# locuslab/icnn

Hardware: AMD Instinct MI355X
Metric: inner-solves/sec (batch x iters), n=159 K=10 (higher is better)
Workload: dtype f32 PICNN / f64 dual solve

## Files before the change

### icnn_amd/csrc/be_common.h

```cpp
#pragma once
#ifndef ICNN_BE_PROF
#define ICNN_BE_PROF 0
#endif
#define ICNN_BE_PROF_ON(p) (ICNN_BE_PROF && (p))
#include <hip/hip_runtime.h>
#include <stdint.h>

namespace icnn_be {

typedef double d4 __attribute__((ext_vector_type(4)));
typedef float f4 __attribute__((ext_vector_type(4)));

constexpr int WAVE = 64;

__device__ __forceinline__ int thread_id() {
    int t = threadIdx.x;
    asm volatile("" : "+v"(t));
    return t;
}

__device__ __forceinline__ int lane_id() { return (int)__builtin_amdgcn_mbcnt_hi(~0u, __builtin_amdgcn_mbcnt_lo(~0u, 0u)); }

__device__ __forceinline__ double wave_sum(double v) {
#pragma unroll
    for (int o = 32; o > 0; o >>= 1) v += __shfl_xor(v, o);
    return v;
}
__device__ __forceinline__ double wave_max(double v) {
#pragma unroll
    for (int o = 32; o > 0; o >>= 1) v = fmax(v, __shfl_xor(v, o));
    return v;
}
__device__ __forceinline__ float wave_sum_f(float v) {
#pragma unroll
    for (int o = 32; o > 0; o >>= 1) v += __shfl_xor(v, o);
    return v;
}

template <int CTRL> __device__ __forceinline__ float dpp_move(float x) {
    return __builtin_bit_cast(float, __builtin_amdgcn_update_dpp(0, __builtin_bit_cast(int, x), CTRL, 0xF, 0xF, true));
}
template <int CTRL> __device__ __forceinline__ double dpp_move(double x) {
    const int lo = __builtin_amdgcn_update_dpp(0, __double2loint(x), CTRL, 0xF, 0xF, true);
    const int hi = __builtin_amdgcn_update_dpp(0, __double2hiint(x), CTRL, 0xF, 0xF, true);
    return __hiloint2double(hi, lo);
}
template <typename T> __device__ __forceinline__ T sum8_numpy_order(T r) {
    r = r + dpp_move<0xB1>(r);
    r = r + dpp_move<0x4E>(r);
    r = r + dpp_move<0x141>(r);
    return r;
}

constexpr int PW_MAX_LEAVES = 64;
constexpr int PW_MAX_PROG = 2 * PW_MAX_LEAVES;
struct PairwisePlan {
    int n_leaves;
    int n_prog;
    int depth;
    short leaf_start[PW_MAX_LEAVES];
    short leaf_len[PW_MAX_LEAVES];
    signed char prog[PW_MAX_PROG];
};

inline void pw_build_rec(PairwisePlan &p, int start, int n, int level) {
    if (n <= 128) {
        p.leaf_start[p.n_leaves] = (short)start;
        p.leaf_len[p.n_leaves] = (short)n;
        p.prog[p.n_prog++] = (signed char)p.n_leaves;
        if (p.n_leaves == 0) p.depth = level;
        else if (p.depth != level) p.depth = -1;
        p.n_leaves++;
        return;
    }
    int n2 = n / 2;
    n2 -= n2 % 8;
    pw_build_rec(p, start, n2, level + 1);
    pw_build_rec(p, start + n2, n - n2, level + 1);
    p.prog[p.n_prog++] = -1;
}
inline bool pw_build(PairwisePlan &p, int n) {
    p.n_leaves = 0;
    p.n_prog = 0;
    p.depth = -1;
    if (n > 128 * PW_MAX_LEAVES / 2) return false;
    pw_build_rec(p, 0, n, 0);
    if (p.depth > 4 || p.n_leaves != (1 << (p.depth < 0 ? 0 : p.depth))) p.depth = -1;
    return true;
}

template <int NW>
__device__ __forceinline__ void sample_sync() {
    if (NW == 1) {
        __builtin_amdgcn_fence(__ATOMIC_SEQ_CST, "wavefront");
        __builtin_amdgcn_wave_barrier();
    } else {
        __syncthreads();
    }
}

template <int NW, typename T, typename Plan, typename Elem>
__device__ void np_pairwise_rows(const Plan &plan, int rows, Elem elem, T *leafbuf, T *out, int tid) {
    const int lane = tid;
    const int grp = tid >> 3, c = tid & 7;
    const int ngrp = (64 * NW) >> 3;
    const int tasks = rows * plan.n_leaves;
    for (int base = 0; base < tasks; base += ngrp) {
        const int task = base + grp;
        const bool live = task < tasks;
        const int r = live ? task / plan.n_leaves : 0;
        const int lf = live ? task - r * plan.n_leaves : 0;
        const int st = plan.leaf_start[lf], len = plan.leaf_len[lf];
        T res = (T)0;
        if (len < 8) {
            for (int i = 0; i < len; ++i) res = res + elem(r, st + i);
        } else {
            const int body = len - (len % 8);
            T acc = elem(r, st + c);
            int i = 8;
            for (; i + 32 <= body; i += 32) {
                const T e0 = elem(r, st + i + c), e1 = elem(r, st + i + 8 + c), e2 = elem(r, st + i + 16 + c),
                        e3 = elem(r, st + i + 24 + c);
                acc = acc + e0;
                acc = acc + e1;
                acc = acc + e2;
                acc = acc + e3;
            }
            for (; i < body; i += 8) acc = acc + elem(r, st + i + c);
            res = sum8_numpy_order(acc);
            for (i = body; i < len; ++i) res = res + elem(r, st + i);
        }
        if (live && c == 0) leafbuf[task] = res;
    }
    sample_sync<NW>();
    if (plan.depth >= 0) {
        const int depth = plan.depth, L = plan.n_leaves, total = rows * L;
        for (int base = 0; base < total; base += 64 * NW) {
            const int t = base + tid;
            T v = t < total ? leafbuf[t] : (T)0;
            if (depth >= 1) v = v + dpp_move<0xB1>(v);
            if (depth >= 2) v = v + dpp_move<0x4E>(v);
            if (depth >= 3) v = v + dpp_move<0x141>(v);
            if (depth >= 4) v = v + dpp_move<0x140>(v);
            if (t < total && (t & (L - 1)) == 0) out[t >> depth] = v;
        }
        sample_sync<NW>();
        return;
    }
    if (lane < rows) {
        T s0 = 0, s1 = 0, s2 = 0, s3 = 0, s4 = 0, s5 = 0, s6 = 0, s7 = 0;
        int sp = 0;
        for (int i = 0; i < plan.n_prog; ++i) {
            const int tok = plan.prog[i];
            if (tok >= 0) {
                const T v = leafbuf[lane * plan.n_leaves + tok];
                switch (sp) {
                case 0: s0 = v; break; case 1: s1 = v; break; case 2: s2 = v; break; case 3: s3 = v; break;
                case 4: s4 = v; break; case 5: s5 = v; break; case 6: s6 = v; break; default: s7 = v; break;
                }
                ++sp;
            } else {
                switch (sp) {
                case 2: s0 = s0 + s1; break; case 3: s1 = s1 + s2; break; case 4: s2 = s2 + s3; break;
                case 5: s3 = s3 + s4; break; case 6: s4 = s4 + s5; break; case 7: s5 = s5 + s6; break;
                default: s6 = s6 + s7; break;
                }
                --sp;
            }
        }
        out[lane] = s0;
    }
    sample_sync<NW>();
}

}
```

### icnn_amd/csrc/be_dual_dev.h

```cpp
#pragma once
#include <hip/hip_runtime.h>
#include <math.h>
#include <type_traits>

#include "be_common.h"
#include "be_kernels.h"
#include "icnn_be.h"

namespace icnn_be {

namespace {

constexpr double BOUND_EPS = 1e-12;
constexpr double ARMIJO_ALPHA = 1e-5;
constexpr double GRAD_TOL = 1e-10;
constexpr double TINY = 1e-10;
constexpr double CYCLE_TOL = 1e-13;
constexpr double NOISE_TOL = 1e-10;
constexpr int NOISE_T0 = 12;
constexpr int ACCEL_T0 = 24;
constexpr int ACCEL_GAP = 6;
constexpr double ACCEL_NEG_RESID = 1e-10;
constexpr double ACCEL_D2MAX = 1e-3;
constexpr double ACCEL_RMAX = 0.98;
// ... 697 lines not shown
        M1[s] = Hm[(i1 < k ? i1 : 0) * HP + jc];
    }
#pragma unroll
    for (int s = 0; s < NS; ++s) { pin(M0[s]); pin(M1[s]); }
#pragma unroll
    for (int s = 0; s < NS; ++s) {
        const int j = 4 * s + q;
        M0[s] = (i0 < k && j < k) ? M0[s] - (j == i0 ? mu : 0.0) : (j == i0 ? 1.0 : 0.0);
        M1[s] = (i1 < k && j < k) ? M1[s] - (j == i1 ? mu : 0.0) : (j == i1 ? 1.0 : 0.0);
    }
    double dp0 = 1.0, dp1 = 1.0;
    static_for<0, KS>([&](auto P) {
        constexpr int p = decltype(P)::value, qp = p & 3, sp = p >> 2, rp = p & 15;
        constexpr bool upper = p >= 16;
        const double d = row_bcast<rp>(upper ? M1[sp] : M0[sp]);
        const double inv = rcp_nr(d);
        double nf0 = 0.0, nf1;
        if constexpr (!upper) {
            dp0 = (q == qp && i0 == p) ? d : dp0;
            nf0 = quarter_bcast<qp>(i0 > p ? -(M0[sp] * inv) : 0.0);
            nf1 = quarter_bcast<qp>(-(M1[sp] * inv));
        } else {
            dp1 = (q == qp && i1 == p) ? d : dp1;
            nf1 = quarter_bcast<qp>(i1 > p ? -(M1[sp] * inv) : 0.0);
        }
        static_for<sp, NS>([&](auto S) {
            constexpr int s = decltype(S)::value;
            const double pr = row_bcast<rp>(upper ? M1[s] : M0[s]);
            if constexpr (!upper) M0[s] = __builtin_fma(nf0, pr, M0[s]);
            M1[s] = __builtin_fma(nf1, pr, M1[s]);
        });
        __builtin_amdgcn_sched_barrier(0);
    });
    const bool own = (r & 3) == q;
    auto fold = [](unsigned long long m) -> unsigned { return (unsigned)((m | (m >> 16) | (m >> 32) | (m >> 48)) & 0xffffull); };
    unsigned nonpos = fold(__ballot(own && !(dp0 > 0.0))) | (fold(__ballot(own && !(dp1 > 0.0))) << 16);
    unsigned zero = fold(__ballot(own && dp0 == 0.0)) | (fold(__ballot(own && dp1 == 0.0)) << 16);
    const unsigned live = k >= 32 ? 0xffffffffu : ((1u << k) - 1u);
    nonpos &= live; zero &= live;
    if (zero) {
        const int p0 = __builtin_ctz(zero);
        return __popc(nonpos & ((2u << p0) - 1u)) + (k - p0 - 1);
    }
    return __popc(nonpos);
}

template <int KT>
__device__ __forceinline__ int inertia_not_above(const double *Hm, int HP, int k, double mu) {
    if (k <= 4) return inertia_not_above_dpp<4>(Hm, HP, k, mu);
    if (k <= 6) return inertia_not_above_dpp<6>(Hm, HP, k, mu);
    if (k <= 8) return inertia_not_above_dpp<8>(Hm, HP, k, mu);
    if (k <= 10) return inertia_not_above_dpp<10>(Hm, HP, k, mu);
    if (k <= 12) return inertia_not_above_dpp<12>(Hm, HP, k, mu);
    if (KT == 16 || k <= 16) return inertia_not_above_dpp<16>(Hm, HP, k, mu);
    if constexpr (KT > 16) {
        if (k <= 20) return inertia_not_above_2d<20>(Hm, HP, k, mu);
        if (k <= 24) return inertia_not_above_2d<24>(Hm, HP, k, mu);
        return inertia_not_above_2d<32>(Hm, HP, k, mu);
    }
    return 0;
}
__device__ __forceinline__ StepResult newton_step_tri(const double *P, int k, int piv, unsigned long long fmask, bool is_free,
                                                      double g0) {
    if (k <= 4) return newton_step_dpp<4, true>(P, 0, k, piv, fmask, is_free, g0);
    if (k <= 6) return newton_step_dpp<6, true>(P, 0, k, piv, fmask, is_free, g0);
    return newton_step_dpp<8, true>(P, 0, k, piv, fmask, is_free, g0);
}
template <int KT>
__device__ __forceinline__ StepResult newton_step(const double *Hm, int HP, int k, int piv, unsigned long long fmask,
                                                  bool is_free, double g0) {
    if (k <= 4) return newton_step_dpp<4>(Hm, HP, k, piv, fmask, is_free, g0);
    if (k <= 6) return newton_step_dpp<6>(Hm, HP, k, piv, fmask, is_free, g0);
    if (k <= 8) return newton_step_dpp<8>(Hm, HP, k, piv, fmask, is_free, g0);
    if (k <= 10) return newton_step_dpp<10>(Hm, HP, k, piv, fmask, is_free, g0);
    if (k <= 12) return newton_step_dpp<12>(Hm, HP, k, piv, fmask, is_free, g0);
    if (KT == 16 || k <= 16) return newton_step_dpp<16>(Hm, HP, k, piv, fmask, is_free, g0);
    if constexpr (KT > 16) {
        if (k <= 20) return newton_step_2d<20>(Hm, HP, k, piv, fmask, is_free, g0);
        if (k <= 24) return newton_step_2d<24>(Hm, HP, k, piv, fmask, is_free, g0);
        return newton_step_2d<32>(Hm, HP, k, piv, fmask, is_free, g0);
    }
    return StepResult{0.0, 0};
}

template <typename Op>
__device__ __forceinline__ double row16_reduce(double v, Op op) {
    v = op(v, dpp_move<0xB1>(v));
    v = op(v, dpp_move<0x4E>(v));
    v = op(v, dpp_move<0x141>(v));
    v = op(v, dpp_move<0x140>(v));
    return uni(v);
}

template <int KT, typename Op>
__device__ __forceinline__ double rows_reduce(double v, int k, Op op) {
    v = op(v, dpp_move<0xB1>(v));
    v = op(v, dpp_move<0x4E>(v));
    v = op(v, dpp_move<0x141>(v));
    v = op(v, dpp_move<0x140>(v));
    if (KT == 16 || k <= 16) return uni(v);
    return op(bcast(v, 0), bcast(v, 16));
}

template <typename CutT, int NC, typename F>
__device__ __forceinline__ void columns_nc(const CutT *As, int ldA, int k, int zrow, int n_pad, int nt, int tid,
                                           double lam, F &&fin) {
    double acc[NC];
    int jc[NC];
#pragma unroll
    for (int c = 0; c < NC; ++c) {
        const int j = tid + c * nt;
        jc[c] = j < n_pad ? j : n_pad - 1;
        acc[c] = 0.0;
    }
    int i0 = 0;
    for (; i0 + 4 <= k; i0 += 4) {
        CutT av[4][NC];
        double li[4];
#pragma unroll
        for (int d = 0; d < 4; ++d) {
            li[d] = bcast(lam, i0 + d);
#pragma unroll
            for (int c = 0; c < NC; ++c) av[d][c] = As[(i0 + d) * ldA + jc[c]];
        }
#pragma unroll
        for (int d = 0; d < 4; ++d)
#pragma unroll
            for (int c = 0; c < NC; ++c) acc[c] += li[d] * (double)av[d][c];
    }
    for (; i0 < k; ++i0) {
        const double li = bcast(lam, i0);
#pragma unroll
        for (int c = 0; c < NC; ++c) acc[c] += li * (double)As[i0 * ldA + jc[c]];
    }
#pragma unroll
    for (int c = 0; c < NC; ++c) fin(tid + c * nt, tid + c * nt < n_pad, acc[c]);
}
template <typename CutT, typename F>
__device__ __forceinline__ void for_columns(const CutT *As, int ldA, int k, int zrow, int n_pad, int nt, int tid,
                                            double lam, F &&fin) {
    const int per_thread = (n_pad + nt - 1) / nt;
    if (per_thread == 3) columns_nc<CutT, 3>(As, ldA, k, zrow, n_pad, nt, tid, lam, fin);
    else if (per_thread <= 2) columns_nc<CutT, 2>(As, ldA, k, zrow, n_pad, nt, tid, lam, fin);
    else if (per_thread == 4) columns_nc<CutT, 4>(As, ldA, k, zrow, n_pad, nt, tid, lam, fin);
    else
        for (int j0 = 0; j0 < n_pad; j0 += 4 * nt)
            columns_nc<CutT, 4>(As + j0, ldA, k, zrow, n_pad - j0, nt, tid, lam,
                                [&](int j, bool valid, double aj) { fin(j0 + j, valid, aj); });
}

#include "be_dual_valu_dev.h"
#include "be_ipm_dev.h"

template <typename CutT, int KT, int NW, bool RL, bool IPM = false, bool GLB = false, int LR = 0, bool SLICED = true, typename ArgsT>
__device__ __forceinline__ void dual_step_body(const ArgsT &a, int u, int tid, unsigned char *smem, int round,
                                               int rows_cap, const CutT *crow_shared) {
    constexpr int NT = 64 * NW;
    const auto &st = a.st;
    const int lane = tid & 63, wave = tid >> 6;
    const bool w0 = wave == 0;
    auto wg_any = [&](bool p) -> bool { return NW == 1 ? (bool)__any(p) : (bool)__syncthreads_or(p); };
    auto combine = [&](double *Hm_, const double *Hp_, int HP_, int k_, int ncols) {
        if (NW == 1) return;
        sample_sync<NW>();
        for (int e = tid; e < k_ * ncols; e += NT) {
            const int r = e / ncols, c = e - r * ncols;
            double acc = 0.0;
            for (int w = 0; w < NW; ++w) acc += Hp_[(w * rows_cap + r) * HP_ + c];
            Hm_[r * HP_ + c] = acc;
        }
    };
    long long tick = ICNN_BE_PROF_ON(a.prof) ? (long long)__builtin_readcyclecounter() : 0;
    const int T = st.slots;
    const int TI = st.iters > 0 ? st.iters : T;
    const int finished_u = st.finished[u], t_raw = st.t_next[u], phase_u = st.phase[u], cnt_raw = st.count[u];
    const int slot_pre = tid < T ? st.active[(size_t)u * T + tid] : 0;
    const int slot_lane = NW == 1 ? slot_pre : (lane < T ? st.active[(size_t)u * T + lane] : 0);
    if (finished_u) return;
    const int t = __builtin_amdgcn_readfirstlane(t_raw);
    if (t >= TI) return;
    const bool resume = SLICED && __builtin_amdgcn_readfirstlane(phase_u) != 0;

    const int n = st.n, n_pad = a.n_pad, ldA = a.ldA;
    const int HP = (rows_cap + 1) | 1;
    static_assert(!IPM || !RL, "interior point is a variant of its own");
    const Carve cv = carve(KT, rows_cap, ldA, n_pad, (int)sizeof(CutT), a.plan.n_leaves, RL, NW, crow_shared == nullptr, IPM, GLB);
    const int cchunk = NW == 1 ? n_pad : (((n_pad / 16 + NW - 1) / NW) * 16);
    const int cbeg = wave * cchunk < n_pad ? wave * cchunk : n_pad;
    const int cend = cbeg + cchunk < n_pad ? cbeg + cchunk : n_pad;
    CutT *As = GLB ? static_cast<CutT *>(st.scratch) + (size_t)u * (st.slots + 2) * ldA : reinterpret_cast<CutT *>(smem + cv.As);
    static_assert(LR == 0 || GLB, "split staging belongs to the device-memory rounds");
    CutT *AsL = reinterpret_cast<CutT *>(smem + ((cv.total + 15) & ~15));
    const bool mirror = LR > 0 && rows_cap <= HV_KMAX;
    double *zs = reinterpret_cast<double *>(smem + cv.zs);
    double *ws = reinterpret_cast<double *>(smem + cv.ws);
    double *sp = reinterpret_cast<double *>(smem + cv.sp);
    double *Hm = reinterpret_cast<double *>(smem + cv.Hm);
    double *Hp = reinterpret_cast<double *>(smem + cv.Hp) + (NW == 1 ? 0 : wave * rows_cap * HP);
    double *Hp0 = reinterpret_cast<double *>(smem + cv.Hp);
    double *leaf = Hm;
    double *psum = Hm + KT * a.plan.n_leaves;
    int *slots = reinterpret_cast<int *>(smem + cv.ints);

    const CutT *g_row = static_cast<const CutT *>(a.g) + (size_t)u * n;
    const double f_u = (sizeof(CutT) == 4 && (st.flags & ICNN_BE_FLAG_F64_ENERGY))
                           ? static_cast<const double *>(a.f)[u] : (double)static_cast<const CutT *>(a.f)[u];
    double *y_row = st.y + (size_t)u * n;
    CutT *G_u = static_cast<CutT *>(st.G) + (size_t)u * T * n;
    double *ys_u = st.ys + (size_t)u * T * n;
    double *h_u = st.h + (size_t)u * T;

    const int cnt = __builtin_amdgcn_readfirstlane(cnt_raw);
    const int k = cnt + 1;
    if (k > rows_cap) {
        if (tid == 0) {
            st.status[u] |= ICNN_BE_ST_OVERFLOW;
            st.finished[u] = 1;
            st.skip_fg[u] = 1;
        }
        return;
    }
    auto lap = [&](int phase) {
        if (ICNN_BE_PROF_ON(a.prof)) {
            const long long now = (long long)__builtin_readcyclecounter();
            if (tid == 0)
                atomicAdd(reinterpret_cast<unsigned long long *>(a.prof) + (size_t)u * DUAL_PROF_PHASES + phase,
                          (unsigned long long)(now - tick));
            tick = now;
        }
    };
    lap(12);
    int slot_new = t;
    if (TI > T) {
        unsigned used = 0;
        for (int i = 0; i < cnt; ++i) used |= 1u << __builtin_amdgcn_readlane(slot_lane, i);
        slot_new = __builtin_ctz(~used);
    }
    if (tid < cnt) slots[tid] = slot_pre;
    if (tid == cnt) slots[tid] = slot_new;
    const double h_old = lane < cnt ? h_u[slot_lane] : 0.0;
    if (NW > 1) sample_sync<NW>();

    const int per_row = (n_pad + NT - 1) / NT;
    constexpr int MAXC = 4;
    auto stage_older = [&]() {
        if constexpr (NW == 1 && !GLB && LR == 0 && sizeof(CutT) == 4) {
            if (per_row <= MAXC) {
                for (int r = 0; r < cnt; ++r) {
                    const CutT *src = G_u + (size_t)uni(slots[r]) * n;
#pragma unroll
                    for (int c = 0; c < MAXC; ++c) {
                        const int j = tid + c * 64;
                        if (c < per_row && j < n)
                            __builtin_amdgcn_global_load_lds((const __attribute__((address_space(1))) void *)(src + j),
                                                             (__attribute__((address_space(3))) void *)(As + r * ldA + c * 64), 4, 0, 0);
                    }
                }
                for (int j = n + tid; j < n_pad; j += 64)
                    for (int r = 0; r < cnt; ++r) As[r * ldA + j] = (CutT)0;
                __builtin_amdgcn_s_waitcnt(0x0f70);
                return;
            }
        }
        if (per_row <= MAXC) {
            constexpr int RB = 4;
            for (int r0 = 0; r0 < cnt; r0 += RB) {
                CutT v[RB][MAXC];
#pragma unroll
                for (int rr = 0; rr < RB; ++rr) {
                    const bool rok = r0 + rr < cnt;
                    const CutT *src = G_u + (size_t)(rok ? slots[r0 + rr] : 0) * n;
#pragma unroll
                    for (int c = 0; c < MAXC; ++c) {
                        const int j = tid + c * NT;
                        v[rr][c] = rok && c < per_row && j < n ? src[j] : (CutT)0;
                    }
                }
#pragma unroll
                for (int rr = 0; rr < RB; ++rr)
#pragma unroll
                    for (int c = 0; c < MAXC; ++c) {
                        const int j = tid + c * NT;
                        if (r0 + rr < cnt && c < per_row && j < n_pad) {
                            As[(r0 + rr) * ldA + j] = v[rr][c];
                            if (LR > 0 && mirror && r0 + rr < LR) AsL[(r0 + rr) * ldA + j] = v[rr][c];
                        }
                    }
            }
            return;
        }
        const int chunks = cnt * per_row;
#pragma unroll 4
        for (int c = 0; c < chunks; ++c) {
            const int r = c / per_row, j = (c - r * per_row) * NT + tid;
            if (j < n_pad) {
                const CutT v = j < n ? G_u[(size_t)slots[r] * n + j] : (CutT)0;
                As[r * ldA + j] = v;
                if (LR > 0 && mirror && r < LR) AsL[r * ldA + j] = v;
            }
        }
    };
    double h_new;
    if (!resume) {
        bool bad = !isfinite(f_u);
        if (per_row <= MAXC) {
            CutT gr[MAXC];
            double yr[MAXC];
#pragma unroll
            for (int c = 0; c < MAXC; ++c) {
                const int j = tid + c * NT;
                gr[c] = j < n ? g_row[j] : (CutT)0;
                yr[c] = j < n ? y_row[j] : 0.0;
            }
            stage_older();
#pragma unroll
            for (int c = 0; c < MAXC; ++c) {
                const int j = tid + c * NT;
                if (j < n) {
                    G_u[(size_t)slot_new * n + j] = gr[c];
                    ys_u[(size_t)slot_new * n + j] = yr[c];
                    bad |= !isfinite((double)gr[c]);
                }
                if (j < n_pad) {
                    As[cnt * ldA + j] = gr[c];
                    if (LR > 0 && mirror && cnt < LR) AsL[cnt * ldA + j] = gr[c];
                    sp[j] = (double)gr[c] * yr[c];
                }
            }
        } else {
            for (int j = tid; j < n_pad; j += NT) {
                double prod = 0.0;
                if (j < n) {
                    const CutT gj = g_row[j];
                    const double yj = y_row[j];
                    G_u[(size_t)slot_new * n + j] = gj;
                    ys_u[(size_t)slot_new * n + j] = yj;
                    prod = (double)gj * yj;
                    bad |= !isfinite((double)gj);
                    As[cnt * ldA + j] = gj;
                    if (LR > 0 && mirror && cnt < LR) AsL[cnt * ldA + j] = gj;
                } else {
                    As[cnt * ldA + j] = (CutT)0;
                    if (LR > 0 && mirror && cnt < LR) AsL[cnt * ldA + j] = (CutT)0;
                }
                sp[j] = prod;
            }
            stage_older();
        }
        sample_sync<NW>();
        lap(13);
        np_pairwise_rows<NW, double>(a.plan, 1, [&](int, int j) { return sp[j]; }, leaf, psum, tid);
        h_new = f_u - psum[0];
        if (tid == 0) {
            h_u[slot_new] = h_new;
            if (st.fvals) st.fvals[(size_t)u * T + slot_new] = f_u;
        }
        if (wg_any(bad)) {
            if (tid == 0) { st.status[u] |= ICNN_BE_ST_NONFINITE; st.finished[u] = 1; st.skip_fg[u] = 1; }
            return;
        }
    } else {
        for (int j = tid; j < n_pad; j += NT) {
            const CutT v = j < n ? G_u[(size_t)slot_new * n + j] : (CutT)0;
            As[cnt * ldA + j] = v;
            if (LR > 0 && mirror && cnt < LR) AsL[cnt * ldA + j] = v;
        }
        h_new = h_u[slot_new];
        stage_older();
    }
    lap(0);
    const CutT *crow = crow_shared ? crow_shared : As + rows_cap * ldA;
    if (!crow_shared)
        for (int j = tid; j < ldA; j += NT) { As[rows_cap * ldA + j] = (CutT)0; As[(rows_cap + 1) * ldA + j] = (CutT)1; }
    const double h_i = lane < cnt ? h_old : h_new;
    const bool hv_on = !(st.flags & ICNN_BE_FLAG_MFMA_CONTRACTION);
    const int hv_p = hv_pitch(k);
    const bool valu = hv_on && (NW > 1 || (n_pad <= 192 && sizeof(CutT) == 4 && k <= HV_K1MAX)) && !RL && !IPM && k >= 2 &&
                      k <= HV_KMAX && (LR == 0 || mirror) && n_pad <= 256 * NW && NW * hv_p <= n_pad;
    double *hv_part = zs;
    const HvEntry hv_first = hv_entry<true>(lane, k, HP);
    sample_sync<NW>();

    lap(1);
    if (!RL && !resume) {
        bool deficient = false;
        const double cfac = (double)(k > n ? k : n) * Cut<CutT>::eps;
        if (k == 1) {
            bool nz = false;
            for (int j = tid; j < n; j += NT) nz |= As[j] != (CutT)0;
            deficient = !wg_any(nz);
        } else if (sizeof(CutT) == 8 && NW == 1) {
            for (int sweep = 0; sweep < 30; ++sweep) {
                bool rotated = false;
                for (int p = 0; p < k - 1; ++p)
                    for (int q = p + 1; q < k; ++q) {
                        double al = 0, be = 0, ga = 0;
                        for (int j = lane; j < n; j += 64) {
                            const double vp = (double)As[p * ldA + j], vq = (double)As[q * ldA + j];
                            al += vp * vp; be += vq * vq; ga += vp * vq;
                        }
                        al = wave_sum(al); be = wave_sum(be); ga = wave_sum(ga);
                        if (ga == 0.0 || fabs(ga) <= 2.3e-16 * sqrt(al * be)) continue;
                        rotated = true;
                        const double zeta = (be - al) / (2.0 * ga);
                        const double tt = zeta != 0.0
                            ? copysign(1.0, zeta) / (fabs(zeta) + sqrt(1.0 + zeta * zeta)) : 1.0;
                        const double c = 1.0 / sqrt(1.0 + tt * tt), s = c * tt;
                        for (int j = lane; j < n; j += 64) {
                            const double vp = (double)As[p * ldA + j], vq = (double)As[q * ldA + j];
                            As[p * ldA + j] = (CutT)(c * vp - s * vq);
                            As[q * ldA + j] = (CutT)(s * vp + c * vq);
                        }
                    }
                if (!rotated) break;
            }
            double sv = 0.0, smax = 0.0;
            for (int r = 0; r < k; ++r) {
                double ss = 0;
                for (int j = lane; j < n; j += 64) { const double v = (double)As[r * ldA + j]; ss += v * v; }
                ss = sqrt(wave_sum(ss));
                if (lane == r) sv = ss;
                smax = fmax(smax, ss);
            }
            deficient = __popcll(__ballot(lane < k && sv > smax * cfac)) < k;
            sample_sync<NW>();
            for (int r = 0; r < k; ++r) {
                const CutT *src = r < cnt ? G_u + (size_t)slots[r] * n : g_row;
                for (int j = lane; j < n_pad; j += 64) As[r * ldA + j] = j < n ? src[j] : (CutT)0;
            }
            sample_sync<NW>();
        } else {
            if (valu) {
                hv_column_pass_k<CutT, NW, false, LR, GLB, (NW == 1 && KT > 16)>(As, AsL, ldA, k, rows_cap, n, n_pad, tid, 0.0, hv_part + wave * hv_p);
                sample_sync<NW>();
                hv_gather<NW, false>(hv_part, hv_p, Hm, HP, k, tid, NT, hv_entry<false>(tid, k, HP));
            } else {
                contract_mfma<CutT, KT, false>(As, ldA, k, crow, cbeg, cend, ws, zs, Hp, HP);
                combine(Hm, Hp0, HP, k, k);
            }
            sample_sync<NW>();
            double trace = 0, total = 0, dmax = 0, rmax = 0;
            {
                double diag = 0, rsum = 0, rabs = 0;
                if (lane < k) {
                    diag = Hm[lane * HP + lane];
                    for (int c = 0; c < k; ++c) { const double v = Hm[lane * HP + c]; rsum += v; rabs += fabs(v); }
                }
                for (int i = 0; i < k; ++i) {
                    const double di = bcast(diag, i);
                    trace += di; dmax = fmax(dmax, di);
                    total += bcast(rsum, i); rmax = fmax(rmax, bcast(rabs, i));
                }
            }
            const double lo = fmax(dmax, total / (double)k);
            const double hi = fmin(trace, rmax);
            const double c2 = cfac * cfac;
            if (inertia_not_above<KT>(Hm, HP, k, c2 * hi) == 0) {
                deficient = false;
            } else if (inertia_not_above<KT>(Hm, HP, k, c2 * lo) > 0) {
                deficient = true;
            } else {
                jacobi_lane0<KT, NW>(Hm, HP, k, tid);
                const double ev = lane < k ? fmax(Hm[lane * HP + lane], 0.0) : 0.0;
                const double svv = sqrt(ev), smax = wave_max(svv);
                deficient = __popcll(__ballot(lane < k && svv > smax * cfac)) < k;
            }
            sample_sync<NW>();
        }
        if (deficient) {
            if (tid == 0) { st.finished[u] = 1; st.n_iters[u] = t - 1; st.skip_fg[u] = 1; }
            return;
        }
    }

    lap(2);
    double lam = 0.0;
    int updates = 0, updates_before = 0;
    if constexpr (IPM) {
        int ipm_status = 0;
        if constexpr (NW > 1) {
            const int kp = k < 2 ? 2 : hv_padded(k);
            const bool waves_ok = sizeof(CutT) == 4 && k <= IPM_KMAX_WAVES && NW * ((ipm_nv(kp) + 3) & ~3) <= n_pad;
            if (waves_ok) {
                lam = ipm_solve_waves<CutT, KT, NW, GLB>(As, ldA, k, n, n_pad, ws, zs, sp, reinterpret_cast<double *>(smem + cv.yv),
                                                    reinterpret_cast<double *>(smem + cv.dv), Hp, HP, h_i, tid, &ipm_status, lap);
            } else {
                if (w0) {
                    lam = ipm_solve<CutT, KT, GLB>(As, ldA, k, crow, n, n_pad, ws, zs, sp, reinterpret_cast<double *>(smem + cv.yv),
                                                   reinterpret_cast<double *>(smem + cv.dv), Hm, HP, h_i, lane, &ipm_status, lap);
                    if (lane == 0) slots[KT - 1] = ipm_status;
                }
                sample_sync<NW>();
                ipm_status = slots[KT - 1];
            }
        } else
        lam = ipm_solve<CutT, KT, GLB>(As, ldA, k, crow, n, n_pad, ws, zs, sp, reinterpret_cast<double *>(smem + cv.yv),
                                  reinterpret_cast<double *>(smem + cv.dv), Hm, HP, h_i, lane, &ipm_status, lap);
        if (ipm_status) {
            if (tid == 0) { st.status[u] |= ICNN_BE_ST_SINGULAR; st.finished[u] = 1; st.skip_fg[u] = 1; }
            return;
        }
    } else if (k == 1) {
        lam = lane == 0 ? 1.0 : 0.0;
    } else {
        CutT *rowsum = reinterpret_cast<CutT *>(psum);
        np_pairwise_rows<NW, CutT>(a.plan, k, [&](int r, int j) { return As[r * ldA + j]; },
                                   reinterpret_cast<CutT *>(leaf), rowsum, tid);
        const double c_i = lane < k ? (double)rowsum[lane] + h_i : 0.0;
        sample_sync<NW>();
        lap(3);
        const int cap = RL ? 20 : 100;
        const int backoff_cap = RL ? 10 : 50;
        const bool shortcut = !(st.flags & ICNN_BE_FLAG_NO_CYCLE_SHORTCUT);
        lam = lane < k ? 1.0 / (double)k : 0.0;
        double prev1 = 0.0, prev2 = 0.0, prev3 = 0.0, prev4 = 0.0;
        int hist = 0, last_jump = -1000;
        double d4_prev = -1.0;
        bool abort_sample = false, parked = false;
        int upd0 = 0;
        double *park = st.park + (size_t)u * (5 * T + 4);
        if (resume) {
            updates = upd0 = updates_before = uni((int)park[5 * T]);
            hist = uni((int)park[5 * T + 1]);
            last_jump = uni((int)park[5 * T + 2]);
            d4_prev = uni(park[5 * T + 3]);
            if (lane < k) {
                lam = park[lane]; prev1 = park[T + lane]; prev2 = park[2 * T + lane]; prev3 = park[3 * T + lane];
                prev4 = park[4 * T + lane];
            }
        }
        int budget = a.budget > 0 ? a.budget : cap;

        while (updates < cap) {
            if (SLICED && budget-- <= 0) { parked = true; break; }
            if (valu) {
                double *part = hv_part + (updates & 1) * (NW * hv_p);
                hv_column_pass_k<CutT, NW, true, LR, GLB, (NW == 1 && KT > 16)>(As, AsL, ldA, k, rows_cap, n, n_pad, tid, lam, part + wave * hv_p);
                sample_sync<NW>();
                lap(4);
                if (NW > 1) hv_gather<NW, true>(part, hv_p, Hp, HP, k, lane, 64, hv_first);
                lap(5);
            } else {
                for_columns<CutT>(As, ldA, k, rows_cap, n_pad, NT, tid, lam, [&](int j, bool valid, double aj) {
                    double z = sigmoid_fast(aj);
                    double w = z * (1.0 - z);
                    if (j >= n) { z = 0.0; w = 0.0; }
                    if (valid) {
                        zs[j] = z;
                        ws[j] = w;
                        if (RL) sp[j] = j < n ? softplus_fast(aj) : 0.0;
                    }
                });
                sample_sync<NW>();
                lap(4);
                contract_mfma<CutT, KT, true>(As, ldA, k, crow, cbeg, cend, ws, zs, Hp, HP, lap);
                combine(Hm, Hp0, HP, k, k + 1);
                sample_sync<NW>();
                lap(5);
            }
            const double *Hq = valu ? Hp : Hm;
            static_assert(HV_K1MAX <= 8 && hv_padded(HV_K1MAX) == HV_K1MAX, "the packed triangle of a k-cut bundle is the k-cut instance's");
            const bool tri = NW == 1 && valu;
            const int hvT = k * (k + 1) / 2;

            const double grad = lane < k ? -c_i + (tri ? hv_part[(updates & 1) * (NW * hv_p) + hvT + lane] : Hq[lane * HP + k]) : 0.0;
            int piv_v = 0;
            {
                const double mx = rows_reduce<KT>(lane < k ? lam : -1e300, k, [](double x, double y) { return fmax(x, y); });
                const unsigned long long at = __ballot(lane < k && lam == mx);
                piv_v = at ? __builtin_ctzll(at) : 0;
            }
            const int piv = __builtin_amdgcn_readfirstlane(piv_v);
            const bool is_piv = lane == piv;
            const double red = is_piv ? 1.0 : lam;
            const double keep = is_piv ? 0.0 : 1.0;
            const double g0 = grad - keep * bcast(grad, piv);
            const bool bound = is_piv || (red <= BOUND_EPS && g0 > 0.0);
            const bool is_free = lane < k && !bound;
            const unsigned long long fmask = __ballot(is_free);
            const double nrm2 = rows_reduce<KT>(is_free ? g0 * g0 : 0.0, k, [](double x, double y) { return x + y; });
            if (sqrt(nrm2) < GRAD_TOL) break;

            lap(8);
            const StepResult sr = tri ? newton_step_tri(hv_part + (updates & 1) * (NW * hv_p), k, piv, fmask, is_free, g0)
                                      : newton_step<KT>(Hq, HP, k, piv, fmask, is_free, g0);
            const double step = sr.step;
            if (!__builtin_amdgcn_readfirstlane(sr.ok)) {
                if (tid == 0) st.status[u] |= ICNN_BE_ST_SINGULAR;
                if (!RL) abort_sample = true;
                break;
            }

            lap(9);
            double tt = 1.0;
            double fval = 0.0, slope = 0.0;
            if (RL) {
                double dmax = 0.0;
                for (int i = 0; i < k; ++i) dmax = fmax(dmax, fabs(bcast(step, i)));
                tt = fmin(1.0 / dmax, 1.0);
                sample_sync<NW>();
                np_pairwise_rows<NW, double>(a.plan, 1, [&](int, int j) { return sp[j]; }, leaf, psum, tid);
                double cl = 0.0;
                for (int i = 0; i < k; ++i) { cl += bcast(c_i * lam, i); slope += bcast(step * g0, i); }
                fval = -cl + psum[0];
                sample_sync<NW>();
            }
            double lam_new = lam;
            bool returned = false;
            for (int bt = 0; bt < backoff_cap; ++bt) {
                const double trial = is_piv ? 1.0 : fmax(red + tt * step, 0.0);
                const double s = rows_reduce<KT>((lane < k && !is_piv) ? trial : 0.0, k,
                                                 [](double x, double y) { return x + y; });
                const double lam_p = 1.0 - s;
                lam_new = lane < k ? (is_piv ? lam_p : trial) : 0.0;
                bool accept = false;
                if (lam_p >= 0.0) {
                    if (RL) {
                        for (int j = tid; j < n_pad; j += NT) {
                            double aj = 0.0;
                            for (int i = 0; i < k; ++i) aj += bcast(lam_new, i) * (double)As[i * ldA + j];
                            sp[j] = j < n ? softplus_fast(aj) : 0.0;
                        }
                        sample_sync<NW>();
                        np_pairwise_rows<NW, double>(a.plan, 1, [&](int, int j) { return sp[j]; }, leaf, psum, tid);
                        double cl = 0.0;
                        for (int i = 0; i < k; ++i) cl += bcast(c_i * lam_new, i);
                        const double f_new = -cl + psum[0];
                        sample_sync<NW>();
                        accept = f_new < fval + tt * ARMIJO_ALPHA * slope;
                    } else {
                        accept = true;
                    }
                }
                if (accept) break;
                if (RL) {
                    double mv = 0.0;
                    for (int i = 0; i < k; ++i) mv = fmax(mv, tt * fabs(bcast(step, i)));
                    if (mv < TINY) { returned = true; break; }
                } else if (tt < TINY) { returned = true; break; }
                tt *= 0.5;
            }
            ++updates;
            if (returned) { lam = lam_new; break; }
            if (shortcut && hist >= 1) {
                if (!__any(fabs(lam_new - prev1) > CYCLE_TOL)) { lam = lam_new; break; }
                if (hist >= 2 && !__any(fabs(lam_new - prev2) > CYCLE_TOL)) {
                    lam = ((cap - updates) & 1) ? prev1 : lam_new;
                    break;
                }
                if (hist >= 3 && !__any(fabs(lam_new - prev3) > CYCLE_TOL)) {
                    const int r = (cap - updates) % 3;
                    lam = r == 0 ? lam_new : (r == 1 ? prev2 : prev1);
                    break;
                }
                if (hist >= 4 && !__any(fabs(lam_new - prev4) > CYCLE_TOL)) {
                    const int r = (cap - updates) & 3;
                    lam = r == 0 ? lam_new : (r == 1 ? prev3 : (r == 2 ? prev2 : prev1));
                    break;
                }
                if (!RL && updates >= NOISE_T0 && hist >= 2) {
                    const bool in = lane < k;
// ... 165 lines not shown
```

### icnn_amd/csrc/be_fused.hip

```cpp
#include "be_dual_dev.h"
#include "be_dual_small_dev.h"
#include "be_picnn_fc_dev.h"
#include "be_picnn_fc_rows_dev.h"

namespace icnn_be {

namespace {

static_assert(NWAVE == TM, "one wave per sample in the dual phase");

struct FusedArgs {
    DualArgs da;
    FcArgs fa;
    int rounds, crow_off, samples_off, sample_bytes;
    int grouped;
    int group_cap, need_off;
    long long *trace;
};
typedef const __attribute__((address_space(4))) FusedArgs KArgs;

template <bool RL, int KT, bool IPM = false, bool SLICED = false>
__global__ __launch_bounds__(NTHREADS) void fused_fc_solve_kernel(FusedArgs args) {
    extern __shared__ __attribute__((aligned(16))) unsigned char smem[];
    KArgs *kp0 = (KArgs *)__builtin_amdgcn_kernarg_segment_ptr();
    {
        float *crow = reinterpret_cast<float *>(smem + args.crow_off);
        for (int j = thread_id(); j < 2 * args.da.ldA; j += NTHREADS) crow[j] = j < args.da.ldA ? 0.f : 1.f;
        if (args.grouped && thread_id() < TM) reinterpret_cast<int *>(smem + args.need_off)[TM + thread_id()] = 0;
    }
    const int rounds = args.rounds;
    for (int r = 0; r < rounds; ++r) {
        KArgs *kp = kp0;
        int tile = blockIdx.x;
        asm volatile("" : "+s"(kp), "+s"(tile));
        fc_fg_tile(kp->fa, tile, reinterpret_cast<float *>(smem));
        __syncthreads();
        int wave = uni(thread_id() >> 6), round = r;
        asm volatile("" : "+s"(kp), "+s"(tile), "+s"(wave), "+s"(round));
        KArgs &k = *kp;
        const int u = tile * k.fa.tile_rows + wave;
        const bool mine = wave < k.fa.tile_rows && u < k.da.st.batch;
        if (!k.grouped) {
            if (mine) {
                const int rows_cap = round + 1 < k.da.st.slots ? round + 1 : k.da.st.slots;
                dual_step_body<float, KT, 1, RL, IPM, false, 0, SLICED>(k.da, u, thread_id() & 63,
                                                                        smem + k.samples_off + wave * k.sample_bytes, round, rows_cap,
                                                                        reinterpret_cast<const float *>(smem + k.crow_off));
            }
            __syncthreads();
            continue;
        }
        int *need = reinterpret_cast<int *>(smem + k.need_off);
        int kk = 0;
        if (mine && k.da.st.finished[u] == 0 && k.da.st.t_next[u] < k.rounds) kk = k.da.st.count[u] + 1;
        kk = uni(kk);
        if (kk > k.da.st.slots) kk = k.da.st.slots;
        if ((thread_id() & 63) == 0)
            need[wave] = kk > 0 ? (carve(KT, kk, k.da.ldA, k.da.n_pad, 4, k.da.plan.n_leaves, RL, 1, false, IPM).total + 15) & ~15 : 0;
        __syncthreads();
        int g = 0, off = 0, my_g = 0, my_off = 0;
        for (int i = 0; i < TM; ++i) {
            const int nb = need[i];
            if (off + nb > k.group_cap) { ++g; off = 0; }
            if (i == wave) { my_g = g; my_off = off; }
            off += nb;
        }
        my_g = uni(my_g); my_off = uni(my_off);
        int alive = kk > 0;
        int *done = need + TM;
        long long tq = ICNN_BE_PROF_ON(k.da.prof) ? (long long)__builtin_readcyclecounter() : 0;
        auto wait_lap = [&](int phase) {
            if (ICNN_BE_PROF_ON(k.da.prof)) {
                const long long now = (long long)__builtin_readcyclecounter();
                if (mine && (thread_id() & 63) == 0)
                    atomicAdd(reinterpret_cast<unsigned long long *>(k.da.prof) + (size_t)u * DUAL_PROF_PHASES + phase,
                              (unsigned long long)(now - tq));
                tq = now;
            }
        };
        long long *tr = nullptr;
        if (ICNN_BE_PROF_ON(k.trace) && kk > 0 && (thread_id() & 63) == 0) {
            tr = k.trace + ((size_t)u * ICNN_BE_MAX_ITERS + round) * DUAL_TRACE_WORDS;
            tr[0] = tq; tr[3] = k.da.st.newton_iters[u];
        }
        if (kk > 0) {
            if (my_g > 0) {
                const int my_end = my_off + need[wave];
                int gi = 0, oi = 0;
                for (int i = 0; i < TM; ++i) {
                    const int nb = need[i];
                    if (oi + nb > k.group_cap) { ++gi; oi = 0; }
                    if (gi >= my_g) break;
                    if (nb > 0 && oi < my_end && oi + nb > my_off)
                        while (__atomic_load_n(&done[i], __ATOMIC_RELAXED) != round + 1) __builtin_amdgcn_s_sleep(4);
                    oi += nb;
                }
                __builtin_amdgcn_fence(__ATOMIC_ACQUIRE, "workgroup");
            }
            wait_lap(14);
            if (ICNN_BE_PROF_ON(k.trace) && tr) tr[1] = (long long)__builtin_readcyclecounter();
            dual_step_body<float, KT, 1, RL, IPM, false, 0, SLICED>(k.da, u, thread_id() & 63, smem + k.samples_off + my_off, round, kk,
                                                                    reinterpret_cast<const float *>(smem + k.crow_off));
            __builtin_amdgcn_fence(__ATOMIC_RELEASE, "workgroup");
            if ((thread_id() & 63) == 0) __atomic_store_n(&done[wave], round + 1, __ATOMIC_RELAXED);
            if (ICNN_BE_PROF_ON(k.da.prof)) tq = (long long)__builtin_readcyclecounter();
            if (ICNN_BE_PROF_ON(k.trace) && tr) tr[2] = (long long)__builtin_readcyclecounter();
        }
        const int any_alive = __syncthreads_or(alive);
        if (kk > 0) wait_lap(15);
        if (!any_alive) break;
    }
}

struct FusedRowsArgs {
    DualArgs da;
    FcArgs fa;
    RowsLayout lay;
    int rounds, per_wg;
    int dual_off, sample_bytes, crow_off;
    int iters;
    int resume;
};
typedef const __attribute__((address_space(4))) FusedRowsArgs KRArgs;

__device__ __forceinline__ void rows_phase_fg(KRArgs *kp, int s_base, int batch, int tid) {
#pragma clang fp contract(off)
    extern __shared__ __attribute__((aligned(16))) unsigned char smem[];
    KRArgs &k = *kp;
    float *lds = reinterpret_cast<float *>(smem);
    const int wave = tid >> 6, lane = tid & 63, n = k.fa.n, RF = k.lay.row_floats;
    long long tick = ICNN_BE_PROF_ON(k.fa.prof) ? (long long)__builtin_readcyclecounter() : 0;
    auto lap = [&](int phase) {
        if (ICNN_BE_PROF_ON(k.fa.prof)) {
            const long long now = (long long)__builtin_readcyclecounter();
            if (lane == 0)
                atomicAdd(reinterpret_cast<unsigned long long *>(k.fa.prof) +
                              ((size_t)blockIdx.x * RWAVES + wave) * FC_PROF_PHASES + phase,
                          (unsigned long long)(now - tick));
            tick = now;
        }
    };
    if (wave < batch)
        for (int j = lane; j < n; j += 64) {
            const double yd = k.da.st.y[(size_t)(s_base + wave) * n + j];
            rows_set_input(k.fa, k.lay, lds + wave * RF, j, k.fa.action_box ? (float)(2.0 * yd - 1.0) : (float)yd);
        }
    __syncthreads();
    lap(13);
    rows_eval(k.fa, k.lay, lds, batch, tid, lap);
    if (wave < batch) {
        const float gscale = k.fa.action_box ? 2.f : 1.f;
        if (lane == 0) k.fa.f[s_base + wave] = lds[k.lay.f_off + wave];
        for (int j = lane; j < n; j += 64) k.fa.g[(size_t)(s_base + wave) * n + j] = gscale * lds[wave * RF + k.lay.g_off + j];
    }
    lap(14);
}

template <bool RL, int KT, int KS = 0, bool IPM = false>
__global__ __launch_bounds__(RTHREADS) void fused_rows_solve_kernel(FusedRowsArgs args) {
    extern __shared__ __attribute__((aligned(16))) unsigned char smem[];
    const int per_wg = args.per_wg;
    int s_base0 = blockIdx.x * per_wg;
    const int batch0 = args.da.st.batch - s_base0 < per_wg ? args.da.st.batch - s_base0 : per_wg;
    KRArgs *kp0 = (KRArgs *)__builtin_amdgcn_kernarg_segment_ptr();
    if (args.resume) {
        int todo = 0;
        if (thread_id() < batch0) {
            const int u = s_base0 + thread_id();
            todo = args.da.st.finished[u] == 0 && args.da.st.t_next[u] < args.iters;
        }
        if (!__syncthreads_or(todo)) return;
    }
    {
        float *crow = reinterpret_cast<float *>(smem + args.crow_off);
        for (int j = thread_id(); j < 2 * args.da.ldA; j += RTHREADS) crow[j] = j < args.da.ldA ? 0.f : 1.f;
    }
    rows_setup(args.fa, args.lay, reinterpret_cast<float *>(smem), s_base0, batch0, thread_id());
    const int rounds = args.rounds;
    for (int r = 0; r < rounds; ++r) {
        KRArgs *kp = kp0;
        int s_base = s_base0, batch = batch0, round = r;
        asm volatile("" : "+s"(kp), "+s"(s_base), "+s"(batch), "+s"(round));
        rows_phase_fg(kp, s_base, batch, thread_id());
        __syncthreads();
        const int wave = uni(thread_id() >> 6);
        asm volatile("" : "+s"(kp), "+s"(s_base), "+s"(batch), "+s"(round));
        KRArgs &k = *kp;
        int live = 0;
        if constexpr (KS > 0) {
            if (wave == 0) {
                dual_step_quad_rl<float, KS>(k.da, s_base, batch, round);
                if ((thread_id() & 63) < batch) live = k.da.st.skip_fg[s_base + (thread_id() & 63)] == 0;
            }
        } else {
            if (wave < batch) {
                const int rows_cap = !k.resume && round + 1 < k.da.st.slots ? round + 1 : k.da.st.slots;
                dual_step_body<float, KT, 1, RL, IPM>(k.da, s_base + wave, thread_id() & 63, smem + k.dual_off + wave * k.sample_bytes,
                                                      round, rows_cap, reinterpret_cast<const float *>(smem + k.crow_off));
            }
            if (wave < batch && (thread_id() & 63) == 0) {
                const int u = s_base + wave;
                live = k.resume ? (k.da.st.finished[u] == 0 && k.da.st.t_next[u] < k.iters) : k.da.st.skip_fg[u] == 0;
            }
        }
        if (!__syncthreads_or(live)) break;
    }
}

}

hipError_t launch_fused_rows_solve(const icnn_be_fc_model &m, const float *ctx, const icnn_be_state &st, float *f_work,
                                   float *g_work, int per_wg, long long *dual_prof, hipStream_t stream, bool resume) {
    const bool rl = st.variant == ICNN_BE_VARIANT_RL;
    const bool ipm = st.variant == ICNN_BE_VARIANT_PDIPM;
    if (st.cut_dtype != ICNN_BE_CUT_F32 || per_wg < 1 || per_wg > ROWS_MAX) return hipErrorNotSupported;
    if (dual_waves(st.n, st.cut_dtype, st.variant) != 1 || (ipm && resume)) return hipErrorNotSupported;
    FusedRowsArgs args{};
    int unused = 0;
    if (fill_args(m, args.fa, unused) != 0) return hipErrorInvalidValue;
    args.fa.ctx = ctx; args.fa.y = st.y; args.fa.f = f_work; args.fa.g = g_work; args.fa.finished = nullptr;
    args.fa.batch = st.batch; args.fa.prof = fc_profile_buffer();
    DualArgs &da = args.da;
    da.st = st;
    da.f = f_work;
    da.g = g_work;
    da.round = 0;
    da.budget = 0;
    da.n_pad = (st.n + 15) & ~15;
    da.ldA = dual_row_pitch(da.n_pad);
    da.rows = st.slots;
    da.prof = dual_prof;
    if (!pw_build(da.plan, st.n)) return hipErrorInvalidValue;
    const bool big = st.slots > 15;
    const int rows_bytes = (rows_layout(m, per_wg, args.lay) + 15) & ~15;
    args.sample_bytes = (carve(big ? 32 : 16, st.slots, da.ldA, da.n_pad, 4, da.plan.n_leaves, rl, 1, false, ipm).total + 15) & ~15;
    args.per_wg = per_wg;
    args.dual_off = rows_bytes;
    args.crow_off = rows_bytes + per_wg * args.sample_bytes;
    const int lds = args.crow_off + ((2 * da.ldA * 4 + 15) & ~15);
    if (lds > 160 * 1024) return hipErrorNotSupported;
    args.rounds = args.iters = st.iters > 0 ? st.iters : st.slots;
    args.resume = resume ? 1 : 0;
    const int which = (rl ? 1 : 0) + (big ? 2 : 0);
    auto kern = which == 0 ? fused_rows_solve_kernel<false, 16> : which == 1 ? fused_rows_solve_kernel<true, 16>
              : which == 2 ? fused_rows_solve_kernel<false, 32> : fused_rows_solve_kernel<true, 32>;
    if (ipm) kern = big ? fused_rows_solve_kernel<false, 32, 0, true> : fused_rows_solve_kernel<false, 16, 0, true>;
    if (!resume && dual_step_small_fits(st, 0))
        kern = st.slots <= 5 ? fused_rows_solve_kernel<true, 16, 5> : st.slots <= 7 ? fused_rows_solve_kernel<true, 16, 8>
                                                                                  : fused_rows_solve_kernel<true, 16, 16>;
    if (hipError_t e = ensure_dynamic_lds(reinterpret_cast<const void *>(kern), lds); e != hipSuccess) return e;
    hipLaunchKernelGGL(kern, dim3((st.batch + per_wg - 1) / per_wg), dim3(RTHREADS), lds, stream, args);
    return hipGetLastError();
}

hipError_t launch_fused_fc_solve(const icnn_be_fc_model &m, const float *ctx, const icnn_be_state &st, float *f_work,
                                 float *g_work, long long *dual_prof, hipStream_t stream, int tile_rows, int budget) {
    const bool rl = st.variant == ICNN_BE_VARIANT_RL, ipm = st.variant == ICNN_BE_VARIANT_PDIPM;
    if (st.cut_dtype != ICNN_BE_CUT_F32) return hipErrorNotSupported;
    if (dual_waves(st.n, st.cut_dtype, st.variant) != 1 || ((ipm || rl) && budget > 0)) return hipErrorNotSupported;
    const bool big = st.slots > 15;
    FcArgs fa{};
    int fg_bytes = 0;
    if (fill_args(m, fa, fg_bytes) != 0) return hipErrorInvalidValue;
    fa.ctx = ctx; fa.y = st.y; fa.f = f_work; fa.g = g_work; fa.finished = st.skip_fg; fa.batch = st.batch;
    fa.prof = nullptr;
    if (tile_rows != 4 && tile_rows != 8 && tile_rows != TM) return hipErrorInvalidValue;
    fa.tile_rows = tile_rows;
    DualArgs da;
    da.st = st;
    da.f = f_work;
    da.g = g_work;
    da.round = 0;
    da.budget = budget;
    da.n_pad = (st.n + 15) & ~15;
    da.ldA = dual_row_pitch(da.n_pad);
    da.rows = st.slots;
    da.prof = dual_prof;
    if (!pw_build(da.plan, st.n)) return hipErrorInvalidValue;
    const int KT = big ? 32 : 16;
    const int sample_bytes = (carve(KT, st.slots, da.ldA, da.n_pad, 4, da.plan.n_leaves, rl, 1, false, ipm).total + 15) & ~15;
    const int samples_off = 0, crow_bytes = (2 * da.ldA * 4 + 15) & ~15;
    const int dual_bytes = samples_off + TM * sample_bytes;
    int crow_off = ((fg_bytes > dual_bytes ? fg_bytes : dual_bytes) + 15) & ~15;
    int lds = crow_off + crow_bytes;
    FusedArgs args;
    args.grouped = 0; args.group_cap = 0; args.need_off = 0;
    if (lds > 160 * 1024 || big) {
        const int need_bytes = 2 * TM * 4;
        crow_off = (160 * 1024 - 1024 - crow_bytes - need_bytes) & ~15;
        if (crow_off < fg_bytes || crow_off < sample_bytes) return hipErrorNotSupported;
        args.grouped = 1; args.group_cap = crow_off; args.need_off = crow_off + crow_bytes;
        lds = args.need_off + need_bytes;
    }
    auto kern = big ? (rl ? fused_fc_solve_kernel<true, 32> : fused_fc_solve_kernel<false, 32>)
                    : (rl ? fused_fc_solve_kernel<true, 16> : fused_fc_solve_kernel<false, 16>);
    if (ipm) kern = big ? fused_fc_solve_kernel<false, 32, true> : fused_fc_solve_kernel<false, 16, true>;
    if (budget > 0) kern = big ? fused_fc_solve_kernel<false, 32, false, true> : fused_fc_solve_kernel<false, 16, false, true>;
    if (hipError_t e = ensure_dynamic_lds(reinterpret_cast<const void *>(kern), lds); e != hipSuccess) return e;
    args.da = da; args.fa = fa; args.trace = dual_trace_buffer();
    args.rounds = st.iters > 0 ? st.iters : st.slots; args.crow_off = crow_off; args.samples_off = samples_off; args.sample_bytes = sample_bytes;
    hipLaunchKernelGGL(kern, dim3((st.batch + tile_rows - 1) / tile_rows), dim3(NTHREADS), lds, stream, args);
    return hipGetLastError();
}

}
```

Baseline: 41.61 million.

## Cache cut row sums alongside h pairwise reduction to skip per-step recomputation

Extends the pairwise-reduction helper to reduce a pair of values, so the row sum of each new cut is computed in the same pass that computes h_new. The result is stored in a per-wave LDS cache indexed by slot. The dual setup then reads cached row sums instead of re-reducing all k cut rows each step. This costs extra LDS per wave and a slightly heavier reduction when a cut is added, and the cached sums must stay consistent with slot reuse.

```diff
diff --git a/icnn_amd/csrc/be_common.h b/icnn_amd/csrc/be_common.h
--- a/icnn_amd/csrc/be_common.h
+++ b/icnn_amd/csrc/be_common.h
@@ -50,6 +50,18 @@
     r = r + dpp_move<0x4E>(r);
     r = r + dpp_move<0x141>(r);
     return r;
+}
+
+template <typename A, typename B> struct SumPair {
+    A a;
+    B b;
+    __device__ SumPair() = default;
+    __device__ constexpr SumPair(int z) : a((A)z), b((B)z) {}
+    __device__ constexpr SumPair(A a_, B b_) : a(a_), b(b_) {}
+    __device__ friend SumPair operator+(const SumPair &x, const SumPair &y) { return SumPair(x.a + y.a, x.b + y.b); }
+};
+template <int CTRL, typename A, typename B> __device__ __forceinline__ SumPair<A, B> dpp_move(SumPair<A, B> x) {
+    return SumPair<A, B>(dpp_move<CTRL>(x.a), dpp_move<CTRL>(x.b));
 }
 
 constexpr int PW_MAX_LEAVES = 64;
diff --git a/icnn_amd/csrc/be_dual_dev.h b/icnn_amd/csrc/be_dual_dev.h
--- a/icnn_amd/csrc/be_dual_dev.h
+++ b/icnn_amd/csrc/be_dual_dev.h
@@ -873,9 +873,10 @@
 #include "be_dual_valu_dev.h"
 #include "be_ipm_dev.h"
 
-template <typename CutT, int KT, int NW, bool RL, bool IPM = false, bool GLB = false, int LR = 0, bool SLICED = true, typename ArgsT>
+template <typename CutT, int KT, int NW, bool RL, bool IPM = false, bool GLB = false, int LR = 0, bool SLICED = true, bool RSC = false,
+          typename ArgsT>
 __device__ __forceinline__ void dual_step_body(const ArgsT &a, int u, int tid, unsigned char *smem, int round,
-                                               int rows_cap, const CutT *crow_shared) {
+                                               int rows_cap, const CutT *crow_shared, CutT *rs_cache = nullptr) {
     constexpr int NT = 64 * NW;
     const auto &st = a.st;
     const int lane = tid & 63, wave = tid >> 6;
@@ -1070,8 +1071,17 @@
         }
         sample_sync<NW>();
         lap(13);
-        np_pairwise_rows<NW, double>(a.plan, 1, [&](int, int j) { return sp[j]; }, leaf, psum, tid);
-        h_new = f_u - psum[0];
+        if constexpr (RSC) {
+            using HS = SumPair<double, CutT>;
+            HS *ps = reinterpret_cast<HS *>(psum);
+            np_pairwise_rows<NW, HS>(a.plan, 1, [&](int, int j) { return HS(sp[j], As[cnt * ldA + j]); },
+                                     reinterpret_cast<HS *>(leaf), ps, tid);
+            h_new = f_u - ps[0].a;
+            if (tid == 0) rs_cache[slot_new] = ps[0].b;
+        } else {
+            np_pairwise_rows<NW, double>(a.plan, 1, [&](int, int j) { return sp[j]; }, leaf, psum, tid);
+            h_new = f_u - psum[0];
+        }
         if (tid == 0) {
             h_u[slot_new] = h_new;
             if (st.fvals) st.fvals[(size_t)u * T + slot_new] = f_u;
@@ -1224,10 +1234,15 @@
     } else if (k == 1) {
         lam = lane == 0 ? 1.0 : 0.0;
     } else {
-        CutT *rowsum = reinterpret_cast<CutT *>(psum);
-        np_pairwise_rows<NW, CutT>(a.plan, k, [&](int r, int j) { return As[r * ldA + j]; },
-                                   reinterpret_cast<CutT *>(leaf), rowsum, tid);
-        const double c_i = lane < k ? (double)rowsum[lane] + h_i : 0.0;
+        double c_i;
+        if constexpr (RSC) {
+            c_i = lane < k ? (double)rs_cache[slots[lane]] + h_i : 0.0;
+        } else {
+            CutT *rowsum = reinterpret_cast<CutT *>(psum);
+            np_pairwise_rows<NW, CutT>(a.plan, k, [&](int r, int j) { return As[r * ldA + j]; },
+                                       reinterpret_cast<CutT *>(leaf), rowsum, tid);
+            c_i = lane < k ? (double)rowsum[lane] + h_i : 0.0;
+        }
         sample_sync<NW>();
         lap(3);
         const int cap = RL ? 20 : 100;
diff --git a/icnn_amd/csrc/be_fused.hip b/icnn_amd/csrc/be_fused.hip
--- a/icnn_amd/csrc/be_fused.hip
+++ b/icnn_amd/csrc/be_fused.hip
@@ -22,6 +22,7 @@
 template <bool RL, int KT, bool IPM = false, bool SLICED = false>
 __global__ __launch_bounds__(NTHREADS) void fused_fc_solve_kernel(FusedArgs args) {
     extern __shared__ __attribute__((aligned(16))) unsigned char smem[];
+    constexpr bool RSC = !IPM;
     KArgs *kp0 = (KArgs *)__builtin_amdgcn_kernarg_segment_ptr();
     {
         float *crow = reinterpret_cast<float *>(smem + args.crow_off);
@@ -40,12 +41,13 @@
         KArgs &k = *kp;
         const int u = tile * k.fa.tile_rows + wave;
         const bool mine = wave < k.fa.tile_rows && u < k.da.st.batch;
+        float *rs_cache = RSC ? reinterpret_cast<float *>(smem + k.crow_off + ((2 * k.da.ldA * 4 + 15) & ~15)) + wave * k.da.st.slots : nullptr;
         if (!k.grouped) {
             if (mine) {
                 const int rows_cap = round + 1 < k.da.st.slots ? round + 1 : k.da.st.slots;
-                dual_step_body<float, KT, 1, RL, IPM, false, 0, SLICED>(k.da, u, thread_id() & 63,
+                dual_step_body<float, KT, 1, RL, IPM, false, 0, SLICED, RSC>(k.da, u, thread_id() & 63,
                                                                         smem + k.samples_off + wave * k.sample_bytes, round, rows_cap,
-                                                                        reinterpret_cast<const float *>(smem + k.crow_off));
+                                                                        reinterpret_cast<const float *>(smem + k.crow_off), rs_cache);
             }
             __syncthreads();
             continue;
@@ -99,8 +101,8 @@
             }
             wait_lap(14);
             if (ICNN_BE_PROF_ON(k.trace) && tr) tr[1] = (long long)__builtin_readcyclecounter();
-            dual_step_body<float, KT, 1, RL, IPM, false, 0, SLICED>(k.da, u, thread_id() & 63, smem + k.samples_off + my_off, round, kk,
-                                                                    reinterpret_cast<const float *>(smem + k.crow_off));
+            dual_step_body<float, KT, 1, RL, IPM, false, 0, SLICED, RSC>(k.da, u, thread_id() & 63, smem + k.samples_off + my_off, round, kk,
+                                                                    reinterpret_cast<const float *>(smem + k.crow_off), rs_cache);
             __builtin_amdgcn_fence(__ATOMIC_RELEASE, "workgroup");
             if ((thread_id() & 63) == 0) __atomic_store_n(&done[wave], round + 1, __ATOMIC_RELAXED);
             if (ICNN_BE_PROF_ON(k.da.prof)) tq = (long long)__builtin_readcyclecounter();
@@ -285,11 +287,13 @@
     int lds = crow_off + crow_bytes;
     FusedArgs args;
     args.grouped = 0; args.group_cap = 0; args.need_off = 0;
+    const int rs_bytes = ipm ? 0 : (TM * st.slots * 4 + 15) & ~15;
+    lds += rs_bytes;
     if (lds > 160 * 1024 || big) {
         const int need_bytes = 2 * TM * 4;
-        crow_off = (160 * 1024 - 1024 - crow_bytes - need_bytes) & ~15;
+        crow_off = (160 * 1024 - 1024 - crow_bytes - need_bytes - rs_bytes) & ~15;
         if (crow_off < fg_bytes || crow_off < sample_bytes) return hipErrorNotSupported;
-        args.grouped = 1; args.group_cap = crow_off; args.need_off = crow_off + crow_bytes;
+        args.grouped = 1; args.group_cap = crow_off; args.need_off = crow_off + crow_bytes + rs_bytes;
         lds = args.need_off + need_bytes;
     }
     auto kern = big ? (rl ? fused_fc_solve_kernel<true, 32> : fused_fc_solve_kernel<false, 32>)
```

Measured after the change: 41.90 million (median of 6 runs). About the same (+0.7%).
